# SarodYatawatta/smart-calibration

Hardware: AMD Instinct MI355X
Metric: env-steps/sec (whole node), elastic-net SAC (higher is better)
Workload: dtype fp32; 1 GPU; model=elasticnet-sac, N=20, M=20, input_dims=420, global_batch=64, replay=1024, reward_scale=20, prioritized=False, parallelism=dp1

## Files before the change

### setup.py

```python

import os
from pathlib import Path

from setuptools import setup

os.environ.setdefault("PYTORCH_ROCM_ARCH", "gfx950")

from torch.utils.cpp_extension import BuildExtension, CUDAExtension

ROOT = Path(__file__).resolve().parent
CSRC = ROOT / "smartcal_amd" / "ops" / "csrc"

sources = [str(CSRC / f) for f in [
    "bindings.hip",
    "fused_linear.hip",
    "gemm_f32.hip",
    "elementwise.hip",
    "enet_solver.hip",
    "als_sweep.hip",
    "conv2d.hip",
    "per.hip",
    "fused_linear_bf16.hip",
    "attention.hip",
    "cgemm.hip",
    "coherency.hip",
    "shapelet.hip",
    "beam.hip",
    "dft_image.hip",
    "hessianres.hip",
    "two_loop.hip",
    "gather_sum.hip",
    "robust.hip",
]]

setup(
    name="smartcal_amd",
    version="0.1.0",
    packages=["smartcal_amd"],
    ext_modules=[
        CUDAExtension(
# ... 11 lines not shown
```

### smartcal_amd/ops/csrc/bindings.hip

```cpp

#include <ATen/hip/HIPContext.h>
#include <c10/hip/HIPStream.h>
#include <torch/extension.h>

#include <algorithm>
#include <climits>
#include <tuple>

#include "common.h"

#define HMAX 7

extern "C" __global__ void fused_linear_fwd_kernel(
    const float*, const float*, const float*, const float*, const float*,
    float*, float*, float*, int, int, int, int, int);
extern "C" __global__ void ln_act_bwd_kernel(const float*, const float*,
                                             const float*, const float*,
                                             const float*, float*, float*,
                                             float*, int, int, int, int,
                                             int);
extern "C" __global__ void gemm_f32_nn_kernel(const float*, const float*,
                                              float*, int, int, int);
extern "C" __global__ void gemm_f32_tn_kernel(const float*, const float*,
                                              float*, float*, int, int, int,
                                              int);
extern "C" __global__ void colsum_kernel(const float*, float*, int, int,
                                         int);
extern "C" __global__ void tanh_gauss_fwd_kernel(const float*, const float*,
                                                 const float*, float*, float*,
                                                 float*, float, int, int);
extern "C" __global__ void tanh_gauss_bwd_kernel(const float*, const float*,
                                                 const float*, const float*,
                                                 const float*, float*, float*,
                                                 float, int, int);
extern "C" __global__ void fused_adam_kernel(float*, const float*, float*,
                                             float*, float*, float, float,
                                             float, float, long);
extern "C" __global__ void adam_bump_kernel(float*);
extern "C" __global__ void enet_lbfgs_solve_kernel(
    const float*, const float*, const float*, float*, float*, float*, int*,
    int, int, int, int, int, int);
extern "C" __global__ void conv2d_k5s2_fwd_kernel(
    const float*, const float*, const float*, float*, int, int, int, int,
    int, int, int);
extern "C" __global__ void conv2d_k5s2_dx_kernel(
    const float*, const float*, float*, int, int, int, int, int, int, int);
extern "C" __global__ void conv2d_k5s2_dw_kernel(
    const float*, const float*, float*, float*, int, int, int, int, int,
    int, int);
struct c32b { float x, y; };
extern "C" __global__ void als_sweep_kernel(
    const c32b*, const c32b*, const c32b*, const int*, const int*,
    const int*, c32b*, c32b*, int, int, int, int, int, int);
extern "C" __global__ void als_sweep_w_kernel(
    const c32b*, const c32b*, const c32b*, const float*, const int*,
    const int*, const int*, c32b*, c32b*, int, int, int, int, int, int);
extern "C" __global__ void vis_residual_weights_kernel(
    const c32b*, const c32b*, const c32b*, const float*, const float*,
    const float*, const int*, const int*, const int*, c32b*, float*, float*,
    double*, int, int, int, int, int);
extern "C" __global__ void enet_influence_kernel(
// ... 782 lines not shown
                at::Tensor& v, at::Tensor& t_dev, double lr, double b1,
                double b2, double eps) {
  check_f32(p, "p");
  check_f32(g, "g");
  check_f32(m, "m");
  check_f32(v, "v");
  check_f32(t_dev, "t_dev");
  const long n = p.numel();
  TORCH_CHECK(g.numel() == n && m.numel() == n && v.numel() == n,
              "fused_adam: g, m and v must hold as many values as p");
  TORCH_CHECK(t_dev.numel() == 1, "fused_adam: t_dev is one step counter");
  if (n == 0) return;
  hipLaunchKernelGGL(fused_adam_kernel, dim3((n + 255) / 256), dim3(256), 0,
                     stream(), p.data_ptr<float>(), g.data_ptr<float>(),
                     m.data_ptr<float>(), v.data_ptr<float>(),
                     t_dev.data_ptr<float>(), (float)lr, (float)b1,
                     (float)b2, (float)eps, n);
  check_launch("fused_adam_kernel");
  hipLaunchKernelGGL(adam_bump_kernel, dim3(1), dim3(64), 0, stream(),
                     t_dev.data_ptr<float>());
  check_launch("adam_bump_kernel");
}

std::tuple<at::Tensor, at::Tensor, at::Tensor, at::Tensor> enet_lbfgs_solve(
    const at::Tensor& A, const at::Tensor& y, const at::Tensor& rho,
    int64_t epochs, int64_t max_iter, int64_t history) {
  check_f32(A, "A");
  check_f32(y, "y");
  check_f32(rho, "rho");
  const int E = A.size(0), N = A.size(1), M = A.size(2);
  TORCH_CHECK(N <= 32 && M <= 32, "enet solver supports N,M <= 32");
  TORCH_CHECK(history <= HMAX, "history <= 7");
  auto x = at::empty({E, M}, A.options());
  auto Y = at::empty({E, (long)HMAX, M}, A.options());
  auto S = at::empty({E, (long)HMAX, M}, A.options());
  auto nh = at::empty({E}, A.options().dtype(at::kInt));
  const int lds_floats = N * M + N + 5 * M + N + 2 * HMAX * M + 2 * M
                         + 2 * HMAX + M;
  hipLaunchKernelGGL(enet_lbfgs_solve_kernel, dim3(E), dim3(64),
                     lds_floats * sizeof(float), stream(),
                     A.data_ptr<float>(), y.data_ptr<float>(),
                     rho.data_ptr<float>(), x.data_ptr<float>(),
                     Y.data_ptr<float>(), S.data_ptr<float>(),
                     nh.data_ptr<int>(), E, N, M, (int)epochs, (int)max_iter,
                     (int)history);
  return {x, Y, S, nh};
// ... 511 lines not shown
}

PYBIND11_MODULE(TORCH_EXTENSION_NAME, m) {
  m.def("fused_linear_fwd", &fused_linear_fwd);
  m.def("fused_linear_bwd_dz", &fused_linear_bwd_dz);
  m.def("mfma_gemm_nn", &mfma_gemm_nn);
  m.def("mfma_gemm_tn_bias", &mfma_gemm_tn_bias);
  m.def("mfma_gemm_tn_bias_into", &mfma_gemm_tn_bias_into);
  m.def("fused_linear_bwd_dz_into", &fused_linear_bwd_dz_into);
  m.def("mlp_chain_fwd", &mlp_chain_fwd, py::arg("x"), py::arg("Ws"),
        py::arg("bs"), py::arg("gammas"), py::arg("betas"), py::arg("acts"),
        py::arg("bf16") = false, py::arg("save") = true);
  m.def("critic_fwd", &critic_fwd, py::arg("state"), py::arg("action"),
        py::arg("Ws"), py::arg("bs"), py::arg("gammas"), py::arg("betas"),
        py::arg("acts"), py::arg("save") = true);
  m.def("als_sweep", &als_sweep);
  m.def("als_sweep_w", &als_sweep_w);
  m.def("vis_residual_weights", &vis_residual_weights);
  m.def("conv2d_k5s2_fwd", &conv2d_k5s2_fwd);
  m.def("conv2d_k5s2_bwd", &conv2d_k5s2_bwd);
  m.def("tanh_gauss_fwd", &tanh_gauss_fwd);
  m.def("tanh_gauss_bwd", &tanh_gauss_bwd);
  m.def("fused_adam", &fused_adam);
  m.def("enet_lbfgs_solve", &enet_lbfgs_solve);
  m.def("enet_influence", &enet_influence);
  m.def("per_sample", &per_sample);
  m.def("per_update", &per_update);
  m.def("fused_linear_bf16_fwd", &fused_linear_bf16_fwd);
  m.def("mfma_gemm_nn_bf16", &mfma_gemm_nn_bf16);
  m.def("mfma_gemm_tn_bias_into_bf16", &mfma_gemm_tn_bias_into_bf16);
  m.def("attn_fwd", &attn_fwd);
  m.def("attn_bwd", &attn_bwd);
  m.def("cgemm_nn_bcast", &cgemm_nn_bcast);
  m.def("coherency_predict", &coherency_predict);
  m.def("shapelet_predict", &shapelet_predict, py::arg("C"),
        py::arg("uvw_scaled"), py::arg("hdr"), py::arg("coff"),
        py::arg("coef"), py::arg("clk"), py::arg("soff"), py::arg("fdelta"),
        py::arg("E") = py::none(), py::arg("p") = py::none(),
        py::arg("q") = py::none(), py::arg("sbase") = 0);
  m.def("station_beam", &station_beam);
  m.def("coherency_beam_predict", &coherency_beam_predict);
  m.def("dft_image", &dft_image, py::arg("uvw"), py::arg("vals"),
        py::arg("fpar"), py::arg("npix"), py::arg("lc"), py::arg("mc"),
        py::arg("nsplit") = 0);
  m.def("hessianres", &hessianres);
  m.def("two_loop_apply", &two_loop_apply);
// ... 3 lines not shown
```

### smartcal_amd/ops/csrc/common.h

```cpp
#pragma once

#include <hip/hip_runtime.h>

#define WAVE 64

template <int CTRL>
__device__ __forceinline__ float _dpp_f(float v) {
  union {
    float f;
    int i;
  } x;
  x.f = v;
  x.i = __builtin_amdgcn_update_dpp(0, x.i, CTRL, 0xF, 0xF, true);
  return x.f;
}

__device__ __forceinline__ float group16_sum(float v) {
  v += _dpp_f<0xB1>(v);
  v += _dpp_f<0x4E>(v);
  v += _dpp_f<0x124>(v);
  v += _dpp_f<0x128>(v);
  return v;
}

// ... 38 lines not shown
  const float* W[CHAIN_LAYERS_MAX];
  const float* bias[CHAIN_LAYERS_MAX];
  const float* gamma[CHAIN_LAYERS_MAX];
  const float* beta[CHAIN_LAYERS_MAX];
  const float* XIN[CHAIN_LAYERS_MAX];
  float* Y[CHAIN_LAYERS_MAX];
  float* ZHAT[CHAIN_LAYERS_MAX];
  float* RSTD[CHAIN_LAYERS_MAX];
  float* YC[CHAIN_LAYERS_MAX];
  int K[CHAIN_LAYERS_MAX];
  int N[CHAIN_LAYERS_MAX];
  int src[CHAIN_LAYERS_MAX];
  int src_off[CHAIN_LAYERS_MAX];
  int dst[CHAIN_LAYERS_MAX];
  int dst_off[CHAIN_LAYERS_MAX];
  int act[CHAIN_LAYERS_MAX];
  int with_ln[CHAIN_LAYERS_MAX];
  int ldc;
  int L;
  int B;
};
#define CHAIN_XMAX 576

#define ACT_NONE 0
#define ACT_ELU 1
#define ACT_RELU 2
#define ACT_TANH 3

__device__ __forceinline__ float apply_act(float h, int act) {
  switch (act) {
    case ACT_ELU:  return h > 0.f ? h : __expf(h) - 1.f;
    case ACT_RELU: return h > 0.f ? h : 0.f;
    case ACT_TANH: return tanhf(h);
    default:       return h;
  }
}

__device__ __forceinline__ float act_grad_from_y(float y, int act) {
  switch (act) {
    case ACT_ELU:  return y > 0.f ? 1.f : y + 1.f;
    case ACT_RELU: return y > 0.f ? 1.f : 0.f;
    case ACT_TANH: return 1.f - y * y;
    default:       return 1.f;
  }
}
```

### smartcal_amd/ops/csrc/elementwise.hip

```cpp

#include "common.h"

#define LOG_SQRT_2PI 0.9189385332046727f
#define REPARAM_NOISE 1e-6f

extern "C" __global__ void tanh_gauss_fwd_kernel(
    const float* __restrict__ MU, const float* __restrict__ LOGSIG,
    const float* __restrict__ EPS, float* __restrict__ ACT,
    float* __restrict__ LOGP, float* __restrict__ AT, float max_action,
    int B, int A) {
  const int row = blockIdx.x;
  const int lane = threadIdx.x;
  float lp = 0.f;
  for (int c = lane; c < A; c += WAVE) {
    const long i = (long)row * A + c;
    const float ls = LOGSIG[i];
    const float sig = expf(ls);
    const float e = EPS[i];
    const float z = MU[i] + sig * e;
    const float at = tanhf(z);
    AT[i] = at;
    ACT[i] = at * max_action;
    lp += -0.5f * e * e - ls - LOG_SQRT_2PI
          - logf(max_action * (1.f - at * at) + REPARAM_NOISE);
  }
  lp = wave_sum(lp);
  if (lane == 0) LOGP[row] = lp;
}

extern "C" __global__ void tanh_gauss_bwd_kernel(
    const float* __restrict__ DACT, const float* __restrict__ DLOGP,
    const float* __restrict__ LOGSIG, const float* __restrict__ EPS,
    const float* __restrict__ AT, float* __restrict__ DMU,
    float* __restrict__ DLOGSIG, float max_action, int B, int A) {
  const long i = (long)blockIdx.x * blockDim.x + threadIdx.x;
  if (i >= (long)B * A) return;
  const int row = i / A;
  const float at = AT[i];
  const float one_m = 1.f - at * at;
  const float sig = expf(LOGSIG[i]);
  const float se = sig * EPS[i];
  const float dl = DLOGP[row];
  const float da = DACT[i];
  const float dlp_dz = 2.f * max_action * at * one_m
                       / (max_action * one_m + REPARAM_NOISE);
  const float dz = da * max_action * one_m + dl * dlp_dz;
  DMU[i] = dz;
  DLOGSIG[i] = dz * se - dl;
}

extern "C" __global__ void fused_adam_kernel(
    float* __restrict__ P, const float* __restrict__ G,
    float* __restrict__ M, float* __restrict__ V, float* __restrict__ tptr,
    float lr, float b1, float b2, float eps, long n) {
  const long i = (long)blockIdx.x * blockDim.x + threadIdx.x;
  const float t = tptr[0] + 1.f;
  if (i >= n) return;
  const float bc1 = 1.f - powf(b1, t);
  const float bc2 = 1.f - powf(b2, t);
  const float g = G[i];
  const float m = b1 * M[i] + (1.f - b1) * g;
  const float v = b2 * V[i] + (1.f - b2) * g * g;
  M[i] = m;
  V[i] = v;
  const float mhat = m / bc1;
  const float vhat = v / bc2;
  P[i] -= lr * mhat / (sqrtf(vhat) + eps);
}

extern "C" __global__ void adam_bump_kernel(float* __restrict__ tptr) {
  if (threadIdx.x == 0 && blockIdx.x == 0) tptr[0] += 1.f;
}
```

### smartcal_amd/ops/sampling.py

```python

from __future__ import annotations

import math
from typing import Optional, Tuple

import torch

from . import ext, use_hip

_LOG_SQRT_2PI = 0.5 * math.log(2.0 * math.pi)
REPARAM_NOISE = 1e-6


class _TanhGaussFn(torch.autograd.Function):
    @staticmethod
    def forward(ctx, mu, logsigma, eps, max_action: float):
        action, logprob, a_t = ext().tanh_gauss_fwd(mu, logsigma, eps,
                                                    max_action)
        ctx.save_for_backward(logsigma, eps, a_t)
        ctx.max_action = max_action
        return action, logprob

    @staticmethod
    def backward(ctx, daction, dlogprob):
        logsigma, eps, a_t = ctx.saved_tensors
        dmu, dlogsigma = ext().tanh_gauss_bwd(
            daction.contiguous(), dlogprob.contiguous(), logsigma, eps, a_t,
            ctx.max_action)
        return dmu, dlogsigma, None, None


def tanh_gauss_sample(mu: torch.Tensor, logsigma: torch.Tensor,
                      max_action: float = 1.0,
                      reparameterize: bool = True,
                      eps: Optional[torch.Tensor] = None
                      ) -> Tuple[torch.Tensor, torch.Tensor]:
    squeeze = mu.dim() == 1
    if squeeze:
        mu = mu.unsqueeze(0)
        logsigma = logsigma.unsqueeze(0)
    if eps is None:
        eps = torch.randn_like(mu)
    else:
        eps = eps.to(mu.dtype).reshape(mu.shape)
    if use_hip(mu):
        mu_c = mu.contiguous()
        logsigma_c = logsigma.contiguous()
        eps_c = eps.contiguous()
        if reparameterize:
            action, logprob = _TanhGaussFn.apply(mu_c, logsigma_c, eps_c,
                                                 float(max_action))
        else:
# ... 18 lines not shown
```

### smartcal_amd/rl/networks.py

```python

from __future__ import annotations

import torch
import torch.nn as nn

from ..ops import use_hip
from ..ops.linear import (FusedLinear, fused_linear, fused_chain,
                          fused_critic, get_compute_dtype)
from ..ops.sampling import tanh_gauss_sample

LOGSIG_MIN = -20.0
LOGSIG_MAX = 2.0

FORCE_COMPOSITION = False


def _one_kernel() -> bool:
    return not FORCE_COMPOSITION and get_compute_dtype() == "fp32"


def _actor_out(net, x: torch.Tensor) -> torch.Tensor:
    if _one_kernel():
        return fused_chain(x, (net.l1, net.l2, net.l3, net.head))
    return net.head(fused_chain(x, (net.l1, net.l2, net.l3)))


class SACActorMLP(nn.Module):
    def __init__(self, input_dim: int, n_actions: int, max_action: float = 1.0):
        super().__init__()
        self.n_actions = n_actions
        self.max_action = max_action
        self.l1 = FusedLinear(input_dim, 512)
        self.l2 = FusedLinear(512, 256)
        self.l3 = FusedLinear(256, 128)
        self.head = FusedLinear(128, 2 * n_actions, ln=False, act="none",
                                init_scale=0.003)

    def forward(self, x: torch.Tensor):
        out = _actor_out(self, x)
        mu = out[..., :self.n_actions]
        logsigma = out[..., self.n_actions:].clamp(LOGSIG_MIN, LOGSIG_MAX)
        return mu, logsigma

    def sample_normal(self, state: torch.Tensor, reparameterize: bool = True):
        mu, logsigma = self.forward(state)
        if mu.dim() == 1:
            mu = mu.unsqueeze(0)
            logsigma = logsigma.unsqueeze(0)
        return tanh_gauss_sample(mu, logsigma, self.max_action,
                                 reparameterize)


class DeterministicActorMLP(nn.Module):

    def __init__(self, input_dim: int, n_actions: int):
        super().__init__()
        self.l1 = FusedLinear(input_dim, 512)
        self.l2 = FusedLinear(512, 256)
        self.l3 = FusedLinear(256, 128)
        self.head = FusedLinear(128, n_actions, ln=False, act="tanh",
                                init_scale=0.003)

    def forward(self, x: torch.Tensor):
        return _actor_out(self, x)


class CriticMLP(nn.Module):
# ... 18 lines not shown
```

### smartcal_amd/rl/sac.py

```python

from __future__ import annotations

import os
from typing import Optional

import numpy as np
import torch
import torch.nn.functional as F

from ..envs.enet import obs_to_state
from ..utils.device import default_device
from ..utils.flatten import FlatParams, FusedAdam
from .buffers import PERBuffer, ReplayBuffer
from .networks import CriticMLP, SACActorMLP


class Agent:
    def __init__(self, gamma, lr_a, lr_c, input_dims, batch_size, n_actions,
                 max_mem_size=100, tau=0.001, reward_scale=2, alpha=0.1,
                 name_prefix="", prioritized=False, use_hint=False,
                 device: Optional[torch.device] = None,
                 checkpoint_dir="./", learn_alpha=False,
                 grad_hook=None):
        self.gamma = gamma
        self.tau = tau
        self.batch_size = batch_size
        self.n_actions = n_actions
        self.max_action = 1.0
        self.min_action = -1.0
        self.prioritized = prioritized
        self.device = device if device is not None else default_device()
        self.checkpoint_dir = checkpoint_dir
        self.name_prefix = name_prefix
        self.grad_hook = grad_hook

        input_dim = input_dims[0] if isinstance(input_dims, (list, tuple)) \
            else int(input_dims)
# ... 105 lines not shown
            self._sync_evs.append(torch.cuda.Event())
        for ev, s in zip(self._sync_evs, self._side_streams):
            ev.record(s)
            ev.wait()

    def _learn_body(self, state_batch, new_state_batch, action_batch,
                    reward_batch, terminal_batch, hint_batch, is_w=None):
        with torch.no_grad():
            new_actions, new_log_probs = self.actor.sample_normal(
                new_state_batch, reparameterize=False)

        def _t1():
            with torch.no_grad():
                return self.target_critic_1(new_state_batch, new_actions)

        def _t2():
            with torch.no_grad():
                return self.target_critic_2(new_state_batch, new_actions)

        q1, q2, q1_t, q2_t = self._fork(
            lambda: self.critic_1(state_batch, action_batch),
            lambda: self.critic_2(state_batch, action_batch),
            _t1, _t2)
        with torch.no_grad():
            min_next_target = torch.min(q1_t, q2_t) \
                - self.alpha * new_log_probs
            min_next_target = min_next_target.masked_fill(terminal_batch,
                                                          0.0)
            new_q_value = reward_batch + self.gamma * min_next_target
        if is_w is not None:
            critic_1_loss = (is_w * (q1 - new_q_value).pow(2)).mean()
            critic_2_loss = (is_w * (q2 - new_q_value).pow(2)).mean()
        else:
            critic_1_loss = F.mse_loss(q1, new_q_value)
            critic_2_loss = F.mse_loss(q2, new_q_value)
        critic_loss = critic_1_loss + critic_2_loss
        self.critic_1_opt.zero_grad()
        self.critic_2_opt.zero_grad()
        critic_loss.backward()
        self._sync_side_streams()
        self._grad_sync([self.critic_1_fp, self.critic_2_fp])
        self._fork(self.critic_1_opt.step, self.critic_2_opt.step)

        actions, log_probs = self.actor.sample_normal(state_batch,
                                                      reparameterize=True)
        for p in self.critic_1.parameters():
            p.requires_grad_(False)
        for p in self.critic_2.parameters():
            p.requires_grad_(False)
        q1_pi, q2_pi = self._pair(
            lambda: self.critic_1(state_batch, actions),
            lambda: self.critic_2(state_batch, actions))
        critic_value = torch.min(q1_pi, q2_pi)

        actor_loss = (self.alpha * log_probs - critic_value).mean()
        if self.use_hint:
            gfun = torch.max(
                self.zero_tensor,
                (F.mse_loss(actions, hint_batch)
                 - self.hint_threshold).mean()).pow(2)
            actor_loss = actor_loss + 0.5 * self.admm_rho * gfun * gfun \
                + self.rho * gfun
        self.actor_opt.zero_grad()
        actor_loss.backward()
        for p in self.critic_1.parameters():
            p.requires_grad_(True)
        for p in self.critic_2.parameters():
            p.requires_grad_(True)
        self._sync_side_streams()
        self._grad_sync([self.actor_fp])
        self.actor_opt.step()
        self.update_network_parameters()
        return q1, new_q_value

    def enable_cuda_graph(self):
        assert not self.use_hint and not self.prioritized
        assert self.device.type == "cuda"
        B = self.batch_size
        mem = self.replaymem
        self._g_idx = torch.zeros(B, dtype=torch.long, device=self.device)
        self._g_state = torch.zeros(B, mem.state_memory.shape[1],
                                    device=self.device)
        self._g_new_state = torch.zeros_like(self._g_state)
        self._g_action = torch.zeros(B, self.n_actions, device=self.device)
        self._g_reward = torch.zeros(B, 1, device=self.device)
        self._g_done = torch.zeros(B, 1, dtype=torch.bool,
                                   device=self.device)
        self._g_hint = torch.zeros(B, self.n_actions, device=self.device)

        n = len(mem)
        if n > 0:
            torch.randint(0, n, (B,), device=self.device, out=self._g_idx)
            torch.index_select(mem.state_memory, 0, self._g_idx,
                               out=self._g_state)
            torch.index_select(mem.new_state_memory, 0, self._g_idx,
                               out=self._g_new_state)
            torch.index_select(mem.action_memory, 0, self._g_idx,
                               out=self._g_action)
            torch.index_select(mem.reward_memory, 0, self._g_idx,
                               out=self._g_reward.view(-1))
            self._g_reward.mul_(self.scale)
            torch.index_select(mem.terminal_memory, 0, self._g_idx,
                               out=self._g_done.view(-1))

        torch.cuda.synchronize()
        s = torch.cuda.Stream()
        s.wait_stream(torch.cuda.current_stream())
        with torch.cuda.stream(s):
            for _ in range(3):
                self._learn_body(self._g_state, self._g_new_state,
                                 self._g_action, self._g_reward,
                                 self._g_done, self._g_hint)
        torch.cuda.current_stream().wait_stream(s)
        torch.cuda.synchronize()

        g = torch.cuda.CUDAGraph()
        with torch.cuda.graph(g):
            self._learn_body(self._g_state, self._g_new_state,
                             self._g_action, self._g_reward,
                             self._g_done, self._g_hint)
        self._graph = g

    def disable_cuda_graph(self):
        self._graph = None

    def _learn_graphed(self):
        mem = self.replaymem
        n = len(mem)
        torch.randint(0, n, (self.batch_size,), device=self.device,
                      out=self._g_idx)
        torch.index_select(mem.state_memory, 0, self._g_idx,
                           out=self._g_state)
        torch.index_select(mem.new_state_memory, 0, self._g_idx,
                           out=self._g_new_state)
        torch.index_select(mem.action_memory, 0, self._g_idx,
                           out=self._g_action)
        torch.index_select(mem.reward_memory, 0, self._g_idx,
                           out=self._g_reward.view(-1))
        self._g_reward.mul_(self.scale)
        torch.index_select(mem.terminal_memory, 0, self._g_idx,
                           out=self._g_done.view(-1))
        self._graph.replay()
        self.learn_counter += 1

    def learn(self):
        if self.replaymem.mem_cntr < self.batch_size:
            return

        if getattr(self, "_graph", None) is not None:
            return self._learn_graphed()

        if self.prioritized:
            (state, action, reward, new_state, done, hint), idxs, is_w = \
                self.replaymem.sample_buffer(self.batch_size)
            is_w = is_w.to(self.device).unsqueeze(1)
        else:
            state, action, reward, new_state, done, hint = \
                self.replaymem.sample_buffer(self.batch_size)
            is_w = None

        state_batch = state.to(self.device)
        new_state_batch = new_state.to(self.device)
        action_batch = action.to(self.device)
        reward_batch = self.scale * reward.to(self.device).unsqueeze(1)
# ... 77 lines not shown
```

### smartcal_amd/utils/flatten.py

```python

from __future__ import annotations

from typing import List

import torch


class FlatParams:

    def __init__(self, module: torch.nn.Module):
        params: List[torch.nn.Parameter] = [p for p in module.parameters()]
        assert params, "module has no parameters"
        device = params[0].device
        dtype = params[0].dtype
        n = sum(p.numel() for p in params)
        self.flat = torch.empty(n, device=device, dtype=dtype)
        self.flat_grad = torch.zeros(n, device=device, dtype=dtype)
        self.params = params
        self.numel = n
        offset = 0
        for p in params:
            k = p.numel()
            self.flat[offset:offset + k].copy_(p.detach().reshape(-1))
            p.data = self.flat[offset:offset + k].view_as(p)
# ... 40 lines not shown

    def zero_grad(self):
        self.fp.zero_grad()

    @torch.no_grad()
    def step(self):
        from ..ops import use_hip, ext
        self.step_count += 1
        t = self.step_count
        g = self.fp.flat_grad
        if self.weight_decay:
            g = g.add(self.fp.flat, alpha=self.weight_decay)
        if use_hip(self.fp.flat):
            ext().fused_adam(self.fp.flat, g, self.m, self.v, self.t_dev,
                             self.lr, self.beta1, self.beta2, self.eps)
        else:
            self.m.mul_(self.beta1).add_(g, alpha=1 - self.beta1)
            self.v.mul_(self.beta2).addcmul_(g, g, value=1 - self.beta2)
            mhat = self.m / (1 - self.beta1 ** t)
            vhat = self.v / (1 - self.beta2 ** t)
            self.fp.flat.addcdiv_(mhat, vhat.sqrt().add_(self.eps),
                                  value=-self.lr)

    def state_dict(self):
        return {"step": self.step_count, "m": self.m, "v": self.v,
                "lr": self.lr, "t_dev": self.t_dev}

    def load_state_dict(self, sd):
        self.step_count = sd["step"]
        self.m.copy_(sd["m"])
        self.v.copy_(sd["v"])
        self.lr = sd.get("lr", self.lr)
        if "t_dev" in sd:
            self.t_dev.copy_(sd["t_dev"])
        else:
            self.t_dev.fill_(float(self.step_count))
```

Baseline: 462.3 env-steps/s.

## Fuse SAC glue ops into custom HIP kernels for losses, Adam+Polyak, replay gather

Adds a set of HIP kernels that fuse the small elementwise steps in the SAC update. These cover the critic and actor loss forward and backward, the tanh-Gaussian head, a paired critic Adam step fused with the target Polyak update, and a single replay-buffer gather that also scales rewards. The aim is to cut kernel launch count and host overhead in a step made of many tiny ops at batch 64. The fused path runs only when there are no importance weights, no hint, and the HIP backend is in use. Moving the Polyak update into the critic optimizer step changes when the target networks are updated relative to the actor step, and the actor target is not touched in this path.

Result: faster. 499.4 env-steps/s (median of 6 runs) (+8.0%).

```diff
diff --git a/setup.py b/setup.py
--- a/setup.py
+++ b/setup.py
@@ -16,6 +16,7 @@
     "fused_linear.hip",
     "gemm_f32.hip",
     "elementwise.hip",
+    "sac_glue.hip",
     "enet_solver.hip",
     "als_sweep.hip",
     "conv2d.hip",
diff --git a/smartcal_amd/ops/csrc/bindings.hip b/smartcal_amd/ops/csrc/bindings.hip
--- a/smartcal_amd/ops/csrc/bindings.hip
+++ b/smartcal_amd/ops/csrc/bindings.hip
@@ -37,6 +37,39 @@
                                              float*, float*, float, float,
                                              float, float, long);
 extern "C" __global__ void adam_bump_kernel(float*);
+extern "C" __global__ void tanh_gauss_head_fwd_kernel(const float*,
+                                                      const float*, float*,
+                                                      float*, float*, float,
+                                                      float, float, int, int);
+extern "C" __global__ void tanh_gauss_head_bwd_kernel(
+    const float*, const float*, const float*, const float*, const float*,
+    float*, float, float, float, int, int);
+extern "C" __global__ void fused_adam_polyak2_kernel(AdamPolyak2Args, float,
+                                                     float, float, float,
+                                                     float, long);
+extern "C" __global__ void adam_bump2_kernel(float*, float*);
+extern "C" __global__ void sac_critic_loss_fwd_kernel(
+    const float*, const float*, const float*, const float*, const float*,
+    const float*, const bool*, const float*, float, float*, float*, int);
+extern "C" __global__ void sac_critic_loss_bwd_kernel(const float*,
+                                                      const float*,
+                                                      const float*,
+                                                      const float*, float,
+                                                      float*, float*, int);
+extern "C" __global__ void sac_actor_loss_fwd_kernel(const float*,
+                                                     const float*,
+                                                     const float*,
+                                                     const float*, float*,
+                                                     int);
+extern "C" __global__ void sac_actor_loss_bwd_kernel(const float*,
+                                                     const float*,
+                                                     const float*,
+                                                     const float*, float,
+                                                     float*, float*, float*,
+                                                     int);
+extern "C" __global__ void replay_gather_kernel(
+    const long*, const float*, const float*, const float*, const float*,
+    const bool*, float, float*, float*, float*, float*, bool*, int, int);
 extern "C" __global__ void enet_lbfgs_solve_kernel(
     const float*, const float*, const float*, float*, float*, float*, int*,
     int, int, int, int, int, int);
@@ -865,6 +898,261 @@
   check_launch("adam_bump_kernel");
 }
 
+std::tuple<at::Tensor, at::Tensor, at::Tensor> tanh_gauss_head_fwd(
+    const at::Tensor& out, const at::Tensor& eps, double max_action,
+    double lo, double hi) {
+  check_f32(out, "out");
+  check_f32(eps, "eps");
+  TORCH_CHECK(out.dim() == 2 && out.size(1) % 2 == 0,
+              "tanh_gauss_head_fwd: out must be (B, 2A)");
+  const int B = out.size(0), A = out.size(1) / 2;
+  TORCH_CHECK(eps.dim() == 2 && eps.size(0) == B && eps.size(1) == A,
+              "tanh_gauss_head_fwd: eps must be (B, A)");
+  auto action = at::empty_like(eps);
+  auto at_ = at::empty_like(eps);
+  auto logp = A == 0 ? at::zeros({B, 1}, out.options())
+                     : at::empty({B, 1}, out.options());
+  if (B == 0 || A == 0) return {action, logp, at_};
+  hipLaunchKernelGGL(tanh_gauss_head_fwd_kernel, dim3(B), dim3(64), 0,
+                     stream(), out.data_ptr<float>(), eps.data_ptr<float>(),
+                     action.data_ptr<float>(), logp.data_ptr<float>(),
+                     at_.data_ptr<float>(), (float)max_action, (float)lo,
+                     (float)hi, B, A);
+  check_launch("tanh_gauss_head_fwd_kernel");
+  return {action, logp, at_};
+}
+
+at::Tensor tanh_gauss_head_bwd(const at::Tensor& dact,
+                               const at::Tensor& dlogp,
+                               const at::Tensor& out, const at::Tensor& eps,
+                               const at::Tensor& at_, double max_action,
+                               double lo, double hi) {
+  check_f32(dact, "dact");
+  check_f32(dlogp, "dlogp");
+  check_f32(out, "out");
+  check_f32(eps, "eps");
+  check_f32(at_, "at");
+  TORCH_CHECK(dact.dim() == 2, "tanh_gauss_head_bwd: dact must be (B, A)");
+  TORCH_CHECK(eps.sizes() == dact.sizes() && at_.sizes() == dact.sizes(),
+              "tanh_gauss_head_bwd: eps and at must have dact's shape");
+  const int B = dact.size(0), A = dact.size(1);
+  TORCH_CHECK(out.dim() == 2 && out.size(0) == B && out.size(1) == 2 * A,
+              "tanh_gauss_head_bwd: out must be (B, 2A)");
+  TORCH_CHECK(dlogp.numel() == B,
+              "tanh_gauss_head_bwd: dlogp must hold B values");
+  auto dout = at::empty_like(out);
+  const long n = (long)B * A;
+  if (n == 0) return dout;
+  hipLaunchKernelGGL(tanh_gauss_head_bwd_kernel, dim3((n + 255) / 256),
+                     dim3(256), 0, stream(), dact.data_ptr<float>(),
+                     dlogp.data_ptr<float>(), out.data_ptr<float>(),
+                     eps.data_ptr<float>(), at_.data_ptr<float>(),
+                     dout.data_ptr<float>(), (float)max_action, (float)lo,
+                     (float)hi, B, A);
+  check_launch("tanh_gauss_head_bwd_kernel");
+  return dout;
+}
+
+void fused_adam_polyak2(at::Tensor& p0, const at::Tensor& g0, at::Tensor& m0,
+                        at::Tensor& v0, at::Tensor& t0, at::Tensor& tgt0,
+                        at::Tensor& p1, const at::Tensor& g1, at::Tensor& m1,
+                        at::Tensor& v1, at::Tensor& t1, at::Tensor& tgt1,
+                        double lr, double b1, double b2, double eps,
+                        double tau) {
+  const at::Tensor* all[] = {&p0, &g0, &m0, &v0, &tgt0,
+                             &p1, &g1, &m1, &v1, &tgt1};
+  const long n = p0.numel();
+  for (const at::Tensor* t : all) {
+    check_f32(*t, "fused_adam_polyak2 pool");
+    TORCH_CHECK(t->numel() == n,
+                "fused_adam_polyak2: every pool must hold as many values as "
+                "p0");
+  }
+  check_f32(t0, "t0");
+  check_f32(t1, "t1");
+  TORCH_CHECK(t0.numel() == 1 && t1.numel() == 1,
+              "fused_adam_polyak2: t0 and t1 are one step counter each");
+  if (n == 0) return;
+  AdamPolyak2Args a;
+  a.P0 = p0.data_ptr<float>();
+  a.P1 = p1.data_ptr<float>();
+  a.G0 = g0.data_ptr<float>();
+  a.G1 = g1.data_ptr<float>();
+  a.M0 = m0.data_ptr<float>();
+  a.M1 = m1.data_ptr<float>();
+  a.V0 = v0.data_ptr<float>();
+  a.V1 = v1.data_ptr<float>();
+  a.t0 = t0.data_ptr<float>();
+  a.t1 = t1.data_ptr<float>();
+  a.T0 = tgt0.data_ptr<float>();
+  a.T1 = tgt1.data_ptr<float>();
+  hipLaunchKernelGGL(fused_adam_polyak2_kernel, dim3((n + 255) / 256, 2),
+                     dim3(256), 0, stream(), a, (float)lr, (float)b1,
+                     (float)b2, (float)eps, (float)tau, n);
+  check_launch("fused_adam_polyak2_kernel");
+  hipLaunchKernelGGL(adam_bump2_kernel, dim3(1), dim3(64), 0, stream(),
+                     t0.data_ptr<float>(), t1.data_ptr<float>());
+  check_launch("adam_bump2_kernel");
+}
+
+inline void check_col(const at::Tensor& t, int64_t B, const char* name) {
+  check_f32(t, name);
+  TORCH_CHECK(t.dim() == 2 && t.size(0) == B && t.size(1) == 1, name,
+              " must be (", B, ", 1), got ", t.sizes());
+}
+
+inline void check_scalar(const at::Tensor& t, const char* name) {
+  check_f32(t, name);
+  TORCH_CHECK(t.numel() == 1, name, " must hold one value");
+}
+
+std::tuple<at::Tensor, at::Tensor> sac_critic_loss_fwd(
+    const at::Tensor& q1, const at::Tensor& q2, const at::Tensor& q1_t,
+    const at::Tensor& q2_t, const at::Tensor& logp, const at::Tensor& reward,
+    const at::Tensor& done, const at::Tensor& alpha, double gamma) {
+  TORCH_CHECK(q1.dim() == 2 && q1.size(0) > 0,
+              "sac_critic_loss_fwd: q1 must be (B, 1) with B > 0");
+  const int64_t B = q1.size(0);
+  check_col(q1, B, "q1");
+  check_col(q2, B, "q2");
+  check_col(q1_t, B, "q1_t");
+  check_col(q2_t, B, "q2_t");
+  check_col(logp, B, "logp");
+  check_col(reward, B, "reward");
+  TORCH_CHECK(done.is_cuda() && done.scalar_type() == at::kBool
+              && done.is_contiguous() && done.numel() == B,
+              "done must hold B contiguous bools on the GPU");
+  check_scalar(alpha, "alpha");
+  auto y = at::empty_like(q1);
+  auto loss = at::empty({}, q1.options());
+  hipLaunchKernelGGL(sac_critic_loss_fwd_kernel, dim3(1), dim3(256), 0,
+                     stream(), q1.data_ptr<float>(), q2.data_ptr<float>(),
+                     q1_t.data_ptr<float>(), q2_t.data_ptr<float>(),
+                     logp.data_ptr<float>(), reward.data_ptr<float>(),
+                     done.data_ptr<bool>(), alpha.data_ptr<float>(),
+                     (float)gamma, y.data_ptr<float>(),
+                     loss.data_ptr<float>(), (int)B);
+  check_launch("sac_critic_loss_fwd_kernel");
+  return {loss, y};
+}
+
+std::tuple<at::Tensor, at::Tensor> sac_critic_loss_bwd(
+    const at::Tensor& q1, const at::Tensor& q2, const at::Tensor& y,
+    const at::Tensor& grad) {
+  TORCH_CHECK(q1.dim() == 2 && q1.size(0) > 0,
+              "sac_critic_loss_bwd: q1 must be (B, 1) with B > 0");
+  const int64_t B = q1.size(0);
+  check_col(q1, B, "q1");
+  check_col(q2, B, "q2");
+  check_col(y, B, "new_q_value");
+  check_scalar(grad, "grad");
+  auto dq1 = at::empty_like(q1);
+  auto dq2 = at::empty_like(q2);
+  hipLaunchKernelGGL(sac_critic_loss_bwd_kernel, dim3((B + 255) / 256),
+                     dim3(256), 0, stream(), q1.data_ptr<float>(),
+                     q2.data_ptr<float>(), y.data_ptr<float>(),
+                     grad.data_ptr<float>(), (float)(2.0 / (double)B),
+                     dq1.data_ptr<float>(), dq2.data_ptr<float>(), (int)B);
+  check_launch("sac_critic_loss_bwd_kernel");
+  return {dq1, dq2};
+}
+
+at::Tensor sac_actor_loss_fwd(const at::Tensor& q1, const at::Tensor& q2,
+                              const at::Tensor& logp,
+                              const at::Tensor& alpha) {
+  TORCH_CHECK(q1.dim() == 2 && q1.size(0) > 0,
+              "sac_actor_loss_fwd: q1 must be (B, 1) with B > 0");
+  const int64_t B = q1.size(0);
+  check_col(q1, B, "q1");
+  check_col(q2, B, "q2");
+  check_col(logp, B, "logp");
+  check_scalar(alpha, "alpha");
+  auto loss = at::empty({}, q1.options());
+  hipLaunchKernelGGL(sac_actor_loss_fwd_kernel, dim3(1), dim3(256), 0,
+                     stream(), q1.data_ptr<float>(), q2.data_ptr<float>(),
+                     logp.data_ptr<float>(), alpha.data_ptr<float>(),
+                     loss.data_ptr<float>(), (int)B);
+  check_launch("sac_actor_loss_fwd_kernel");
+  return loss;
+}
+
+std::tuple<at::Tensor, at::Tensor, at::Tensor> sac_actor_loss_bwd(
+    const at::Tensor& q1, const at::Tensor& q2, const at::Tensor& alpha,
+    const at::Tensor& grad) {
+  TORCH_CHECK(q1.dim() == 2 && q1.size(0) > 0,
+              "sac_actor_loss_bwd: q1 must be (B, 1) with B > 0");
+  const int64_t B = q1.size(0);
+  check_col(q1, B, "q1");
+  check_col(q2, B, "q2");
+  check_scalar(alpha, "alpha");
+  check_scalar(grad, "grad");
+  auto dq1 = at::empty_like(q1);
+  auto dq2 = at::empty_like(q1);
+  auto dlogp = at::empty_like(q1);
+  hipLaunchKernelGGL(sac_actor_loss_bwd_kernel, dim3((B + 255) / 256),
+                     dim3(256), 0, stream(), q1.data_ptr<float>(),
+                     q2.data_ptr<float>(), alpha.data_ptr<float>(),
+                     grad.data_ptr<float>(), 1.0f / (float)B,
+                     dq1.data_ptr<float>(), dq2.data_ptr<float>(),
+                     dlogp.data_ptr<float>(), (int)B);
+  check_launch("sac_actor_loss_bwd_kernel");
+  return {dq1, dq2, dlogp};
+}
+
+void replay_gather(const at::Tensor& idx, const at::Tensor& state_mem,
+                   const at::Tensor& new_state_mem,
+                   const at::Tensor& action_mem,
+                   const at::Tensor& reward_mem,
+                   const at::Tensor& terminal_mem, double scale,
+                   at::Tensor& out_state, at::Tensor& out_new_state,
+                   at::Tensor& out_action, at::Tensor& out_reward,
+                   at::Tensor& out_done) {
+  check_f32(state_mem, "state_mem");
+  check_f32(new_state_mem, "new_state_mem");
+  check_f32(action_mem, "action_mem");
+  check_f32(reward_mem, "reward_mem");
+  check_f32(out_state, "out_state");
+  check_f32(out_new_state, "out_new_state");
+  check_f32(out_action, "out_action");
+  check_f32(out_reward, "out_reward");
+  TORCH_CHECK(out_state.dim() >= 1, "replay_gather: out_state must be (B, D)");
+  const int64_t B = out_state.size(0);
+  check_index(idx, at::kLong, B, "idx");
+  TORCH_CHECK(state_mem.dim() >= 1 && state_mem.size(0) > 0,
+              "replay_gather: state_mem must have rows");
+  const int64_t rows = state_mem.size(0);
+  const int64_t D = state_mem.numel() / rows;
+  const int64_t A = action_mem.numel() / rows;
+  TORCH_CHECK(new_state_mem.numel() == rows * D
+              && action_mem.numel() == rows * A
+              && reward_mem.numel() == rows && terminal_mem.numel() == rows,
+              "replay_gather: the memories must have the same number of rows");
+  TORCH_CHECK(terminal_mem.is_cuda() && terminal_mem.scalar_type() == at::kBool
+              && terminal_mem.is_contiguous(),
+              "terminal_mem must be contiguous bools on the GPU");
+  TORCH_CHECK(out_done.is_cuda() && out_done.scalar_type() == at::kBool
+              && out_done.is_contiguous() && out_done.numel() == B,
+              "out_done must hold B contiguous bools on the GPU");
+  TORCH_CHECK(out_state.numel() == B * D && out_new_state.numel() == B * D
+              && out_action.numel() == B * A && out_reward.numel() == B,
+              "replay_gather: the outputs must be B rows of the memories' "
+              "widths");
+  if (B == 0) return;
+  hipLaunchKernelGGL(replay_gather_kernel, dim3(B), dim3(256), 0, stream(),
+                     (const long*)idx.data_ptr<int64_t>(),
+                     state_mem.data_ptr<float>(),
+                     new_state_mem.data_ptr<float>(),
+                     action_mem.data_ptr<float>(),
+                     reward_mem.data_ptr<float>(),
+                     terminal_mem.data_ptr<bool>(), (float)scale,
+                     out_state.data_ptr<float>(),
+                     out_new_state.data_ptr<float>(),
+                     out_action.data_ptr<float>(),
+                     out_reward.data_ptr<float>(),
+                     out_done.data_ptr<bool>(), (int)D, (int)A);
+  check_launch("replay_gather_kernel");
+}
+
 std::tuple<at::Tensor, at::Tensor, at::Tensor, at::Tensor> enet_lbfgs_solve(
     const at::Tensor& A, const at::Tensor& y, const at::Tensor& rho,
     int64_t epochs, int64_t max_iter, int64_t history) {
@@ -1422,6 +1710,14 @@
   m.def("tanh_gauss_fwd", &tanh_gauss_fwd);
   m.def("tanh_gauss_bwd", &tanh_gauss_bwd);
   m.def("fused_adam", &fused_adam);
+  m.def("tanh_gauss_head_fwd", &tanh_gauss_head_fwd);
+  m.def("tanh_gauss_head_bwd", &tanh_gauss_head_bwd);
+  m.def("fused_adam_polyak2", &fused_adam_polyak2);
+  m.def("sac_critic_loss_fwd", &sac_critic_loss_fwd);
+  m.def("sac_critic_loss_bwd", &sac_critic_loss_bwd);
+  m.def("sac_actor_loss_fwd", &sac_actor_loss_fwd);
+  m.def("sac_actor_loss_bwd", &sac_actor_loss_bwd);
+  m.def("replay_gather", &replay_gather);
   m.def("enet_lbfgs_solve", &enet_lbfgs_solve);
   m.def("enet_influence", &enet_influence);
   m.def("per_sample", &per_sample);
diff --git a/smartcal_amd/ops/csrc/common.h b/smartcal_amd/ops/csrc/common.h
--- a/smartcal_amd/ops/csrc/common.h
+++ b/smartcal_amd/ops/csrc/common.h
@@ -84,6 +84,15 @@
 };
 #define CHAIN_XMAX 576
 
+struct AdamPolyak2Args {
+  float *P0, *P1;
+  const float *G0, *G1;
+  float *M0, *M1;
+  float *V0, *V1;
+  const float *t0, *t1;
+  float *T0, *T1;
+};
+
 #define ACT_NONE 0
 #define ACT_ELU 1
 #define ACT_RELU 2
diff --git a/smartcal_amd/ops/csrc/elementwise.hip b/smartcal_amd/ops/csrc/elementwise.hip
--- a/smartcal_amd/ops/csrc/elementwise.hip
+++ b/smartcal_amd/ops/csrc/elementwise.hip
@@ -3,6 +3,19 @@
 
 #define LOG_SQRT_2PI 0.9189385332046727f
 #define REPARAM_NOISE 1e-6f
+
+__device__ __forceinline__ float tanh_gauss_elem(float mu, float ls, float e,
+                                                 float max_action,
+                                                 float* __restrict__ at_out,
+                                                 float* __restrict__ act_out) {
+  const float sig = expf(ls);
+  const float z = mu + sig * e;
+  const float at = tanhf(z);
+  *at_out = at;
+  *act_out = at * max_action;
+  return -0.5f * e * e - ls - LOG_SQRT_2PI
+         - logf(max_action * (1.f - at * at) + REPARAM_NOISE);
+}
 
 extern "C" __global__ void tanh_gauss_fwd_kernel(
     const float* __restrict__ MU, const float* __restrict__ LOGSIG,
@@ -14,15 +27,30 @@
   float lp = 0.f;
   for (int c = lane; c < A; c += WAVE) {
     const long i = (long)row * A + c;
-    const float ls = LOGSIG[i];
-    const float sig = expf(ls);
-    const float e = EPS[i];
-    const float z = MU[i] + sig * e;
-    const float at = tanhf(z);
-    AT[i] = at;
-    ACT[i] = at * max_action;
-    lp += -0.5f * e * e - ls - LOG_SQRT_2PI
-          - logf(max_action * (1.f - at * at) + REPARAM_NOISE);
+    lp += tanh_gauss_elem(MU[i], LOGSIG[i], EPS[i], max_action, &AT[i],
+                          &ACT[i]);
+  }
+  lp = wave_sum(lp);
+  if (lane == 0) LOGP[row] = lp;
+}
+
+__device__ __forceinline__ float clamp_nan(float v, float lo, float hi) {
+  return v != v ? v : fminf(fmaxf(v, lo), hi);
+}
+
+extern "C" __global__ void tanh_gauss_head_fwd_kernel(
+    const float* __restrict__ OUT, const float* __restrict__ EPS,
+    float* __restrict__ ACT, float* __restrict__ LOGP,
+    float* __restrict__ AT, float max_action, float lo, float hi, int B,
+    int A) {
+  const int row = blockIdx.x;
+  const int lane = threadIdx.x;
+  const float* o = OUT + (long)row * 2 * A;
+  float lp = 0.f;
+  for (int c = lane; c < A; c += WAVE) {
+    const long i = (long)row * A + c;
+    lp += tanh_gauss_elem(o[c], clamp_nan(o[A + c], lo, hi), EPS[i],
+                          max_action, &AT[i], &ACT[i]);
   }
   lp = wave_sum(lp);
   if (lane == 0) LOGP[row] = lp;
@@ -49,6 +77,49 @@
   DLOGSIG[i] = dz * se - dl;
 }
 
+extern "C" __global__ void tanh_gauss_head_bwd_kernel(
+    const float* __restrict__ DACT, const float* __restrict__ DLOGP,
+    const float* __restrict__ OUT, const float* __restrict__ EPS,
+    const float* __restrict__ AT, float* __restrict__ DOUT, float max_action,
+    float lo, float hi, int B, int A) {
+#pragma clang fp contract(off)
+  const long i = (long)blockIdx.x * blockDim.x + threadIdx.x;
+  if (i >= (long)B * A) return;
+  const int row = i / A;
+  const int c = i - (long)row * A;
+  const long j = (long)row * 2 * A + A + c;
+  const float raw = OUT[j];
+  const float at = AT[i];
+  const float one_m = __builtin_fmaf(-at, at, 1.f);
+  const float sig = expf(clamp_nan(raw, lo, hi));
+  const float se = sig * EPS[i];
+  const float dl = DLOGP[row];
+  const float da = DACT[i];
+  const float dlp_dz = 2.f * max_action * at * one_m
+                       / (max_action * one_m + REPARAM_NOISE);
+  const float dz = da * max_action * one_m + dl * dlp_dz;
+  DOUT[j - A] = dz + 0.f;
+  DOUT[j] = (raw >= lo && raw <= hi) ? __builtin_fmaf(dz, se, -dl) + 0.f
+                                     : 0.f;
+}
+
+__device__ __forceinline__ float adam_elem(float p, float g,
+                                           float* __restrict__ M,
+                                           float* __restrict__ V, float t,
+                                           float lr, float b1, float b2,
+                                           float eps) {
+  const float bc1 = 1.f - powf(b1, t);
+  const float bc2 = 1.f - powf(b2, t);
+  const float m = b1 * *M + (1.f - b1) * g;
+  const float v = b2 * *V + (1.f - b2) * g * g;
+  *M = m;
+  *V = v;
+  const float mhat = m / bc1;
+  const float vhat = v / bc2;
+  p -= lr * mhat / (sqrtf(vhat) + eps);
+  return p;
+}
+
 extern "C" __global__ void fused_adam_kernel(
     float* __restrict__ P, const float* __restrict__ G,
     float* __restrict__ M, float* __restrict__ V, float* __restrict__ tptr,
@@ -56,18 +127,40 @@
   const long i = (long)blockIdx.x * blockDim.x + threadIdx.x;
   const float t = tptr[0] + 1.f;
   if (i >= n) return;
-  const float bc1 = 1.f - powf(b1, t);
-  const float bc2 = 1.f - powf(b2, t);
-  const float g = G[i];
-  const float m = b1 * M[i] + (1.f - b1) * g;
-  const float v = b2 * V[i] + (1.f - b2) * g * g;
-  M[i] = m;
-  V[i] = v;
-  const float mhat = m / bc1;
-  const float vhat = v / bc2;
-  P[i] -= lr * mhat / (sqrtf(vhat) + eps);
+  P[i] = adam_elem(P[i], G[i], &M[i], &V[i], t, lr, b1, b2, eps);
 }
 
 extern "C" __global__ void adam_bump_kernel(float* __restrict__ tptr) {
   if (threadIdx.x == 0 && blockIdx.x == 0) tptr[0] += 1.f;
 }
+
+__device__ __forceinline__ float lerp_torch(float a, float b, float w) {
+  const float d = b - a;
+  return fabsf(w) < 0.5f ? __fmaf_rn(w, d, a) : __fmaf_rn(-d, 1.f - w, b);
+}
+
+extern "C" __global__ void fused_adam_polyak2_kernel(AdamPolyak2Args a,
+                                                     float lr, float b1,
+                                                     float b2, float eps,
+                                                     float tau, long n) {
+  const long i = (long)blockIdx.x * blockDim.x + threadIdx.x;
+  const int k = blockIdx.y;
+  float* __restrict__ P = k ? a.P1 : a.P0;
+  const float* __restrict__ G = k ? a.G1 : a.G0;
+  float* __restrict__ M = k ? a.M1 : a.M0;
+  float* __restrict__ V = k ? a.V1 : a.V0;
+  float* __restrict__ T = k ? a.T1 : a.T0;
+  const float t = (k ? a.t1 : a.t0)[0] + 1.f;
+  if (i >= n) return;
+  const float p = adam_elem(P[i], G[i], &M[i], &V[i], t, lr, b1, b2, eps);
+  P[i] = p;
+  T[i] = lerp_torch(T[i], p, tau);
+}
+
+extern "C" __global__ void adam_bump2_kernel(float* __restrict__ t0,
+                                             float* __restrict__ t1) {
+  if (threadIdx.x == 0 && blockIdx.x == 0) {
+    t0[0] += 1.f;
+    t1[0] += 1.f;
+  }
+}
diff --git a/smartcal_amd/ops/csrc/sac_glue.hip b/smartcal_amd/ops/csrc/sac_glue.hip
--- /dev/null
+++ b/smartcal_amd/ops/csrc/sac_glue.hip
@@ -0,0 +1,105 @@
+
+#include "common.h"
+
+#pragma clang fp contract(off)
+
+#define LOSS_THREADS 256
+
+__device__ __forceinline__ float minimum_nan(float a, float b) {
+  return a != a ? a : (b != b ? b : fminf(a, b));
+}
+
+__device__ __forceinline__ float block_sum(float v, float* red) {
+  v = wave_sum(v);
+  if ((threadIdx.x & (WAVE - 1)) == 0) red[threadIdx.x / WAVE] = v;
+  __syncthreads();
+  float s = 0.f;
+  if (threadIdx.x == 0)
+    for (int w = 0; w < LOSS_THREADS / WAVE; ++w) s += red[w];
+  __syncthreads();
+  return s;
+}
+
+extern "C" __global__ void sac_critic_loss_fwd_kernel(
+    const float* __restrict__ Q1, const float* __restrict__ Q2,
+    const float* __restrict__ Q1T, const float* __restrict__ Q2T,
+    const float* __restrict__ LOGP, const float* __restrict__ R,
+    const bool* __restrict__ DONE, const float* __restrict__ ALPHA,
+    float gamma, float* __restrict__ Y, float* __restrict__ LOSS, int B) {
+  __shared__ float red[LOSS_THREADS / WAVE];
+  const float alpha = ALPHA[0];
+  float s1 = 0.f, s2 = 0.f;
+  for (int i = threadIdx.x; i < B; i += LOSS_THREADS) {
+    float t = minimum_nan(Q1T[i], Q2T[i]) - alpha * LOGP[i];
+    t = DONE[i] ? 0.f : t;
+    const float y = R[i] + gamma * t;
+    Y[i] = y;
+    const float d1 = Q1[i] - y, d2 = Q2[i] - y;
+    s1 += d1 * d1;
+    s2 += d2 * d2;
+  }
+  s1 = block_sum(s1, red);
+  s2 = block_sum(s2, red);
+  if (threadIdx.x == 0) LOSS[0] = s1 / (float)B + s2 / (float)B;
+}
+
+extern "C" __global__ void sac_critic_loss_bwd_kernel(
+    const float* __restrict__ Q1, const float* __restrict__ Q2,
+    const float* __restrict__ Y, const float* __restrict__ GRAD, float norm,
+    float* __restrict__ DQ1, float* __restrict__ DQ2, int B) {
+  const int i = blockIdx.x * blockDim.x + threadIdx.x;
+  if (i >= B) return;
+  const float g = GRAD[0], y = Y[i];
+  DQ1[i] = norm * (Q1[i] - y) * g;
+  DQ2[i] = norm * (Q2[i] - y) * g;
+}
+
+extern "C" __global__ void sac_actor_loss_fwd_kernel(
+    const float* __restrict__ Q1, const float* __restrict__ Q2,
+    const float* __restrict__ LOGP, const float* __restrict__ ALPHA,
+    float* __restrict__ LOSS, int B) {
+  __shared__ float red[LOSS_THREADS / WAVE];
+  const float alpha = ALPHA[0];
+  float s = 0.f;
+  for (int i = threadIdx.x; i < B; i += LOSS_THREADS)
+    s += alpha * LOGP[i] - minimum_nan(Q1[i], Q2[i]);
+  s = block_sum(s, red);
+  if (threadIdx.x == 0) LOSS[0] = s / (float)B;
+}
+
+extern "C" __global__ void sac_actor_loss_bwd_kernel(
+    const float* __restrict__ Q1, const float* __restrict__ Q2,
+    const float* __restrict__ ALPHA, const float* __restrict__ GRAD,
+    float inv_b, float* __restrict__ DQ1, float* __restrict__ DQ2,
+    float* __restrict__ DLOGP, int B) {
+  const int i = blockIdx.x * blockDim.x + threadIdx.x;
+  if (i >= B) return;
+  const float c = GRAD[0] * inv_b;
+  const float q1 = Q1[i], q2 = Q2[i];
+  const float d = q1 == q2 ? -c / 2.f : -c;
+  DLOGP[i] = c * ALPHA[0];
+  DQ1[i] = q1 > q2 ? 0.f : d;
+  DQ2[i] = q1 < q2 ? 0.f : d;
+}
+
+extern "C" __global__ void replay_gather_kernel(
+    const long* __restrict__ IDX, const float* __restrict__ STATE,
+    const float* __restrict__ NEW_STATE, const float* __restrict__ ACTION,
+    const float* __restrict__ REWARD, const bool* __restrict__ TERMINAL,
+    float scale, float* __restrict__ OUT_STATE,
+    float* __restrict__ OUT_NEW_STATE, float* __restrict__ OUT_ACTION,
+    float* __restrict__ OUT_REWARD, bool* __restrict__ OUT_DONE, int D,
+    int A) {
+  const long b = blockIdx.x;
+  const long r = IDX[b];
+  for (int c = threadIdx.x; c < D; c += blockDim.x) {
+    OUT_STATE[b * D + c] = STATE[r * D + c];
+    OUT_NEW_STATE[b * D + c] = NEW_STATE[r * D + c];
+  }
+  for (int c = threadIdx.x; c < A; c += blockDim.x)
+    OUT_ACTION[b * A + c] = ACTION[r * A + c];
+  if (threadIdx.x == 0) {
+    OUT_REWARD[b] = REWARD[r] * scale;
+    OUT_DONE[b] = TERMINAL[r];
+  }
+}
diff --git a/smartcal_amd/ops/sampling.py b/smartcal_amd/ops/sampling.py
--- a/smartcal_amd/ops/sampling.py
+++ b/smartcal_amd/ops/sampling.py
@@ -28,6 +28,47 @@
             daction.contiguous(), dlogprob.contiguous(), logsigma, eps, a_t,
             ctx.max_action)
         return dmu, dlogsigma, None, None
+
+
+class _TanhGaussHeadFn(torch.autograd.Function):
+    @staticmethod
+    def forward(ctx, out, eps, max_action: float, lo: float, hi: float):
+        action, logprob, a_t = ext().tanh_gauss_head_fwd(out, eps,
+                                                         max_action, lo, hi)
+        ctx.save_for_backward(out, eps, a_t)
+        ctx.consts = (max_action, lo, hi)
+        return action, logprob
+
+    @staticmethod
+    def backward(ctx, daction, dlogprob):
+        out, eps, a_t = ctx.saved_tensors
+        dout = ext().tanh_gauss_head_bwd(
+            daction.contiguous(), dlogprob.contiguous(), out, eps, a_t,
+            *ctx.consts)
+        return dout, None, None, None, None
+
+
+def tanh_gauss_head_sample(out: torch.Tensor, lo: float, hi: float,
+                           max_action: float = 1.0,
+                           reparameterize: bool = True,
+                           eps: Optional[torch.Tensor] = None
+                           ) -> Tuple[torch.Tensor, torch.Tensor]:
+    if out.dim() == 1:
+        out = out.unsqueeze(0)
+    mu = out[..., :out.shape[-1] // 2]
+    if eps is None:
+        eps = torch.randn_like(mu)
+    else:
+        eps = eps.to(mu.dtype).reshape(mu.shape)
+    out_c = out.contiguous()
+    eps_c = eps.contiguous()
+    if reparameterize:
+        return _TanhGaussHeadFn.apply(out_c, eps_c, float(max_action),
+                                      float(lo), float(hi))
+    with torch.no_grad():
+        action, logprob, _ = ext().tanh_gauss_head_fwd(
+            out_c, eps_c, float(max_action), float(lo), float(hi))
+    return action, logprob
 
 
 def tanh_gauss_sample(mu: torch.Tensor, logsigma: torch.Tensor,
diff --git a/smartcal_amd/rl/networks.py b/smartcal_amd/rl/networks.py
--- a/smartcal_amd/rl/networks.py
+++ b/smartcal_amd/rl/networks.py
@@ -7,7 +7,7 @@
 from ..ops import use_hip
 from ..ops.linear import (FusedLinear, fused_linear, fused_chain,
                           fused_critic, get_compute_dtype)
-from ..ops.sampling import tanh_gauss_sample
+from ..ops.sampling import tanh_gauss_head_sample, tanh_gauss_sample
 
 LOGSIG_MIN = -20.0
 LOGSIG_MAX = 2.0
@@ -43,6 +43,11 @@
         return mu, logsigma
 
     def sample_normal(self, state: torch.Tensor, reparameterize: bool = True):
+        from . import sac
+        if use_hip(state) and not sac.FORCE_TORCH_GLUE:
+            return tanh_gauss_head_sample(_actor_out(self, state),
+                                          LOGSIG_MIN, LOGSIG_MAX,
+                                          self.max_action, reparameterize)
         mu, logsigma = self.forward(state)
         if mu.dim() == 1:
             mu = mu.unsqueeze(0)
diff --git a/smartcal_amd/rl/sac.py b/smartcal_amd/rl/sac.py
--- a/smartcal_amd/rl/sac.py
+++ b/smartcal_amd/rl/sac.py
@@ -9,10 +9,59 @@
 import torch.nn.functional as F
 
 from ..envs.enet import obs_to_state
+from ..ops import ext, use_hip
 from ..utils.device import default_device
 from ..utils.flatten import FlatParams, FusedAdam
 from .buffers import PERBuffer, ReplayBuffer
 from .networks import CriticMLP, SACActorMLP
+
+FORCE_TORCH_GLUE = False
+
+
+class _CriticLossFn(torch.autograd.Function):
+    @staticmethod
+    def forward(ctx, q1, q2, q1_t, q2_t, logp_next, reward, done, alpha,
+                gamma: float):
+        loss, new_q_value = ext().sac_critic_loss_fwd(
+            q1, q2, q1_t, q2_t, logp_next, reward, done, alpha, gamma)
+        ctx.save_for_backward(q1, q2, new_q_value)
+        ctx.mark_non_differentiable(new_q_value)
+        ctx.set_materialize_grads(False)
+        return loss, new_q_value
+
+    @staticmethod
+    def backward(ctx, g, _):
+        q1, q2, new_q_value = ctx.saved_tensors
+        dq1, dq2 = ext().sac_critic_loss_bwd(q1, q2, new_q_value,
+                                             g.contiguous())
+        return dq1, dq2, None, None, None, None, None, None, None
+
+
+def sac_critic_loss(q1, q2, q1_t, q2_t, logp_next, reward, done, alpha,
+                    gamma):
+    return _CriticLossFn.apply(
+        q1.contiguous(), q2.contiguous(), q1_t.contiguous(),
+        q2_t.contiguous(), logp_next.contiguous(), reward.contiguous(),
+        done.contiguous(), alpha, float(gamma))
+
+
+class _ActorLossFn(torch.autograd.Function):
+    @staticmethod
+    def forward(ctx, q1_pi, q2_pi, logp, alpha):
+        ctx.save_for_backward(q1_pi, q2_pi, alpha)
+        return ext().sac_actor_loss_fwd(q1_pi, q2_pi, logp, alpha)
+
+    @staticmethod
+    def backward(ctx, g):
+        q1_pi, q2_pi, alpha = ctx.saved_tensors
+        dq1, dq2, dlogp = ext().sac_actor_loss_bwd(q1_pi, q2_pi, alpha,
+                                                   g.contiguous())
+        return dq1, dq2, dlogp, None
+
+
+def sac_actor_loss(q1_pi, q2_pi, logp, alpha):
+    return _ActorLossFn.apply(q1_pi.contiguous(), q2_pi.contiguous(),
+                              logp.contiguous(), alpha)
 
 
 class Agent:
@@ -164,25 +213,37 @@
             lambda: self.critic_1(state_batch, action_batch),
             lambda: self.critic_2(state_batch, action_batch),
             _t1, _t2)
-        with torch.no_grad():
-            min_next_target = torch.min(q1_t, q2_t) \
-                - self.alpha * new_log_probs
-            min_next_target = min_next_target.masked_fill(terminal_batch,
-                                                          0.0)
-            new_q_value = reward_batch + self.gamma * min_next_target
-        if is_w is not None:
-            critic_1_loss = (is_w * (q1 - new_q_value).pow(2)).mean()
-            critic_2_loss = (is_w * (q2 - new_q_value).pow(2)).mean()
+        native = (is_w is None and not self.use_hint
+                  and not FORCE_TORCH_GLUE and use_hip(q1))
+        if native:
+            critic_loss, new_q_value = sac_critic_loss(
+                q1, q2, q1_t, q2_t, new_log_probs, reward_batch,
+                terminal_batch, self.alpha, self.gamma)
         else:
-            critic_1_loss = F.mse_loss(q1, new_q_value)
-            critic_2_loss = F.mse_loss(q2, new_q_value)
-        critic_loss = critic_1_loss + critic_2_loss
+            with torch.no_grad():
+                min_next_target = torch.min(q1_t, q2_t) \
+                    - self.alpha * new_log_probs
+                min_next_target = min_next_target.masked_fill(
+                    terminal_batch, 0.0)
+                new_q_value = reward_batch + self.gamma * min_next_target
+            if is_w is not None:
+                critic_1_loss = (is_w * (q1 - new_q_value).pow(2)).mean()
+                critic_2_loss = (is_w * (q2 - new_q_value).pow(2)).mean()
+            else:
+                critic_1_loss = F.mse_loss(q1, new_q_value)
+                critic_2_loss = F.mse_loss(q2, new_q_value)
+            critic_loss = critic_1_loss + critic_2_loss
         self.critic_1_opt.zero_grad()
         self.critic_2_opt.zero_grad()
         critic_loss.backward()
         self._sync_side_streams()
         self._grad_sync([self.critic_1_fp, self.critic_2_fp])
-        self._fork(self.critic_1_opt.step, self.critic_2_opt.step)
+        if native:
+            FusedAdam.step_pair_polyak(
+                self.critic_1_opt, self.critic_2_opt,
+                self.target_critic_1_fp, self.target_critic_2_fp, self.tau)
+        else:
+            self._fork(self.critic_1_opt.step, self.critic_2_opt.step)
 
         actions, log_probs = self.actor.sample_normal(state_batch,
                                                       reparameterize=True)
@@ -193,9 +254,11 @@
         q1_pi, q2_pi = self._pair(
             lambda: self.critic_1(state_batch, actions),
             lambda: self.critic_2(state_batch, actions))
-        critic_value = torch.min(q1_pi, q2_pi)
-
-        actor_loss = (self.alpha * log_probs - critic_value).mean()
+        if native:
+            actor_loss = sac_actor_loss(q1_pi, q2_pi, log_probs, self.alpha)
+        else:
+            critic_value = torch.min(q1_pi, q2_pi)
+            actor_loss = (self.alpha * log_probs - critic_value).mean()
         if self.use_hint:
             gfun = torch.max(
                 self.zero_tensor,
@@ -212,7 +275,8 @@
         self._sync_side_streams()
         self._grad_sync([self.actor_fp])
         self.actor_opt.step()
-        self.update_network_parameters()
+        if not native:
+            self.update_network_parameters()
         return q1, new_q_value
 
     def enable_cuda_graph(self):
@@ -232,18 +296,7 @@
 
         n = len(mem)
         if n > 0:
-            torch.randint(0, n, (B,), device=self.device, out=self._g_idx)
-            torch.index_select(mem.state_memory, 0, self._g_idx,
-                               out=self._g_state)
-            torch.index_select(mem.new_state_memory, 0, self._g_idx,
-                               out=self._g_new_state)
-            torch.index_select(mem.action_memory, 0, self._g_idx,
-                               out=self._g_action)
-            torch.index_select(mem.reward_memory, 0, self._g_idx,
-                               out=self._g_reward.view(-1))
-            self._g_reward.mul_(self.scale)
-            torch.index_select(mem.terminal_memory, 0, self._g_idx,
-                               out=self._g_done.view(-1))
+            self._sample_statics(n)
 
         torch.cuda.synchronize()
         s = torch.cuda.Stream()
@@ -263,14 +316,17 @@
                              self._g_done, self._g_hint)
         self._graph = g
 
-    def disable_cuda_graph(self):
-        self._graph = None
-
-    def _learn_graphed(self):
+    def _sample_statics(self, n):
         mem = self.replaymem
-        n = len(mem)
         torch.randint(0, n, (self.batch_size,), device=self.device,
                       out=self._g_idx)
+        if not FORCE_TORCH_GLUE:
+            ext().replay_gather(
+                self._g_idx, mem.state_memory, mem.new_state_memory,
+                mem.action_memory, mem.reward_memory, mem.terminal_memory,
+                float(self.scale), self._g_state, self._g_new_state,
+                self._g_action, self._g_reward, self._g_done)
+            return
         torch.index_select(mem.state_memory, 0, self._g_idx,
                            out=self._g_state)
         torch.index_select(mem.new_state_memory, 0, self._g_idx,
@@ -282,6 +338,12 @@
         self._g_reward.mul_(self.scale)
         torch.index_select(mem.terminal_memory, 0, self._g_idx,
                            out=self._g_done.view(-1))
+
+    def disable_cuda_graph(self):
+        self._graph = None
+
+    def _learn_graphed(self):
+        self._sample_statics(len(self.replaymem))
         self._graph.replay()
         self.learn_counter += 1
 
diff --git a/smartcal_amd/utils/flatten.py b/smartcal_amd/utils/flatten.py
--- a/smartcal_amd/utils/flatten.py
+++ b/smartcal_amd/utils/flatten.py
@@ -86,6 +86,24 @@
             self.fp.flat.addcdiv_(mhat, vhat.sqrt().add_(self.eps),
                                   value=-self.lr)
 
+    @staticmethod
+    @torch.no_grad()
+    def step_pair_polyak(opt_a: "FusedAdam", opt_b: "FusedAdam",
+                         target_a: FlatParams, target_b: FlatParams,
+                         tau: float):
+        from ..ops import ext
+        hyper = (opt_a.lr, opt_a.beta1, opt_a.beta2, opt_a.eps)
+        assert hyper == (opt_b.lr, opt_b.beta1, opt_b.beta2, opt_b.eps) \
+            and not opt_a.weight_decay and not opt_b.weight_decay, \
+            "step_pair_polyak: the two optimizers must be configured alike"
+        opt_a.step_count += 1
+        opt_b.step_count += 1
+        ext().fused_adam_polyak2(
+            opt_a.fp.flat, opt_a.fp.flat_grad, opt_a.m, opt_a.v, opt_a.t_dev,
+            target_a.flat,
+            opt_b.fp.flat, opt_b.fp.flat_grad, opt_b.m, opt_b.v, opt_b.t_dev,
+            target_b.flat, *hyper, float(tau))
+
     def state_dict(self):
         return {"step": self.step_count, "m": self.m, "v": self.v,
                 "lr": self.lr, "t_dev": self.t_dev}
```
